# Artemarius/cuda-gaussian-splatting

Measured on AMD Instinct MI355X. Metric: fwd+bwd Mpixels/s @1080p, 1M Gaussians, SH3, higher is better.
Workload: dtype f32

## Files before the change

### cuda-gaussian-splatting_amd/csrc/cugs_gaussian_math.h

```cpp
#pragma once

#include "cugs_common.h"

struct V3 { float x, y, z; };
struct Sym2 { float a, b, c; };
struct Sym3 { float xx, xy, xz, yy, yz, zz; };
struct M3 { float m00, m01, m02, m10, m11, m12, m20, m21, m22; };
struct M23 { float r0x, r0y, r0z, r1x, r1y, r1z; };

struct GradMoments { float m1x, m1y, m2xx, m2xy, m2yy; };
struct Grad2D { float mx, my, a, b, c; };
__device__ __forceinline__ Grad2D grads_from_moments(const GradMoments& m, float a, float b, float c) {
    Grad2D g;
    g.mx = a * m.m1x + b * m.m1y;
    g.my = b * m.m1x + c * m.m1y;
    g.a = -0.5f * m.m2xx;
    g.b = -m.m2xy;
    g.c = -0.5f * m.m2yy;
    return g;
}

__device__ __forceinline__ M3 view_rotation(const CamArgs& c) {
    return M3{c.view[0], c.view[1], c.view[2], c.view[4], c.view[5], c.view[6],
              c.view[8], c.view[9], c.view[10]};
}

__device__ __forceinline__ V3 to_camera(const CamArgs& c, const M3& W, V3 p) {
    V3 t;
    t.x = W.m00 * p.x + W.m01 * p.y + W.m02 * p.z + c.view[3];
    t.y = W.m10 * p.x + W.m11 * p.y + W.m12 * p.z + c.view[7];
    t.z = W.m20 * p.x + W.m21 * p.y + W.m22 * p.z + c.view[11];
    return t;
}

struct QuatRot { M3 R; float inv_norm, w, x, y, z; };
__device__ __forceinline__ QuatRot rotation_of(float w, float x, float y, float z) {
    QuatRot o;
    o.inv_norm = cugs_rsqrtf(w * w + x * x + y * y + z * z + 1e-12f);
    w *= o.inv_norm; x *= o.inv_norm; y *= o.inv_norm; z *= o.inv_norm;
    o.w = w; o.x = x; o.y = y; o.z = z;
    o.R.m00 = 1.0f - 2.0f * (y * y + z * z);
    o.R.m01 = 2.0f * (x * y - w * z);
    o.R.m02 = 2.0f * (x * z + w * y);
    o.R.m10 = 2.0f * (x * y + w * z);
    o.R.m11 = 1.0f - 2.0f * (x * x + z * z);
    o.R.m12 = 2.0f * (y * z - w * x);
    o.R.m20 = 2.0f * (x * z - w * y);
    o.R.m21 = 2.0f * (y * z + w * x);
    o.R.m22 = 1.0f - 2.0f * (x * x + y * y);
    return o;
}

__device__ __forceinline__ M3 scale_columns(const M3& R, V3 s) {
    return M3{R.m00 * s.x, R.m01 * s.y, R.m02 * s.z, R.m10 * s.x, R.m11 * s.y, R.m12 * s.z,
              R.m20 * s.x, R.m21 * s.y, R.m22 * s.z};
}

__device__ __forceinline__ Sym3 gram(const M3& M) {
    Sym3 S;
    S.xx = M.m00 * M.m00 + M.m01 * M.m01 + M.m02 * M.m02;
    S.xy = M.m00 * M.m10 + M.m01 * M.m11 + M.m02 * M.m12;
    S.xz = M.m00 * M.m20 + M.m01 * M.m21 + M.m02 * M.m22;
    S.yy = M.m10 * M.m10 + M.m11 * M.m11 + M.m12 * M.m12;
    S.yz = M.m10 * M.m20 + M.m11 * M.m21 + M.m12 * M.m22;
    S.zz = M.m20 * M.m20 + M.m21 * M.m21 + M.m22 * M.m22;
    return S;
}

struct Jac { float j00, j02, j11, j12, tz_inv, tz_inv2; };
__device__ __forceinline__ Jac jacobian(V3 t, float fx, float fy) {
    Jac J;
    J.tz_inv = 1.0f / (t.z + 1e-6f);
    J.tz_inv2 = J.tz_inv * J.tz_inv;
    J.j00 = fx * J.tz_inv;
    J.j02 = -fx * t.x * J.tz_inv2;
    J.j11 = fy * J.tz_inv;
    J.j12 = -fy * t.y * J.tz_inv2;
    return J;
}

__device__ __forceinline__ M23 project_matrix_full(const Jac& J, const M3& W) {
    const float z = 0.0f;
    M23 T;
    T.r0x = J.j00 * W.m00 + z * W.m10 + J.j02 * W.m20;
    T.r0y = J.j00 * W.m01 + z * W.m11 + J.j02 * W.m21;
    T.r0z = J.j00 * W.m02 + z * W.m12 + J.j02 * W.m22;
    T.r1x = z * W.m00 + J.j11 * W.m10 + J.j12 * W.m20;
    T.r1y = z * W.m01 + J.j11 * W.m11 + J.j12 * W.m21;
    T.r1z = z * W.m02 + J.j11 * W.m12 + J.j12 * W.m22;
    return T;
}

__device__ __forceinline__ M23 project_matrix_sparse(const Jac& J, const M3& W) {
    M23 T;
    T.r0x = J.j00 * W.m00 + J.j02 * W.m20;
    T.r0y = J.j00 * W.m01 + J.j02 * W.m21;
    T.r0z = J.j00 * W.m02 + J.j02 * W.m22;
    T.r1x = J.j11 * W.m10 + J.j12 * W.m20;
    T.r1y = J.j11 * W.m11 + J.j12 * W.m21;
    T.r1z = J.j11 * W.m12 + J.j12 * W.m22;
    return T;
}

__device__ __forceinline__ M23 times_sym3(const M23& T, const Sym3& S) {
    M23 P;
    P.r0x = T.r0x * S.xx + T.r0y * S.xy + T.r0z * S.xz;
    P.r0y = T.r0x * S.xy + T.r0y * S.yy + T.r0z * S.yz;
    P.r0z = T.r0x * S.xz + T.r0y * S.yz + T.r0z * S.zz;
    P.r1x = T.r1x * S.xx + T.r1y * S.xy + T.r1z * S.xz;
    P.r1y = T.r1x * S.xy + T.r1y * S.yy + T.r1z * S.yz;
    P.r1z = T.r1x * S.xz + T.r1y * S.yz + T.r1z * S.zz;
    return P;
}

__device__ __forceinline__ Sym2 screen_covariance(const M23& T, const Sym3& S) {
    M23 P = times_sym3(T, S);
    Sym2 c;
    c.a = P.r0x * T.r0x + P.r0y * T.r0y + P.r0z * T.r0z;
    c.b = P.r0x * T.r1x + P.r0y * T.r1y + P.r0z * T.r1z;
    c.c = P.r1x * T.r1x + P.r1y * T.r1y + P.r1z * T.r1z;
    c.a += 0.3f;
    c.c += 0.3f;
    return c;
}

__device__ __forceinline__ int splat_radius(const Sym2& c) {
    float det = c.a * c.c - c.b * c.b;
    float trace = c.a + c.c;
    float disc = fmaxf(trace * trace - 4.0f * det, 0.0f);
    float lambda_max = 0.5f * (trace + sqrtf(disc));
    if (lambda_max <= 0.0f) return 0;
    return cugs_f2i(ceilf(3.0f * sqrtf(lambda_max)));
}

__device__ __forceinline__ float invert_sym2(const Sym2& c, Sym2& inv) {
    float det = c.a * c.c - c.b * c.b;
    if (det <= 0.0f) { inv = Sym2{0.0f, 0.0f, 0.0f}; return 0.0f; }
    float inv_det = 1.0f / det;
    inv.a = c.c * inv_det;
    inv.b = -c.b * inv_det;
    inv.c = c.a * inv_det;
    return det;
}

struct TileRect { int x0, y0, x1, y1; };
__device__ __forceinline__ TileRect tile_rect_of(float x, float y, int radius, int w, int h,
                                                 int ntx, int nty) {
    float rf = (float)radius;
    int min_x = max(0, cugs_f2i(x - rf));
    int min_y = max(0, cugs_f2i(y - rf));
    int max_x = min(w, cugs_f2i(x + rf + 1.0f));
    int max_y = min(h, cugs_f2i(y + rf + 1.0f));
    TileRect r;
    r.x0 = min_x / CUGS_TILE;
    r.y0 = min_y / CUGS_TILE;
    r.x1 = min(ntx, (max_x + CUGS_TILE - 1) / CUGS_TILE);
    r.y1 = min(nty, (max_y + CUGS_TILE - 1) / CUGS_TILE);
    return r;
}

constexpr int CUGS_DEPTH_BITS = 9;
constexpr uint32_t CUGS_DEPTH_KEY_BASE = 0x3E4CCCCCu;
constexpr uint32_t CUGS_DEPTH_KEY_SPAN = 1u << (3 * CUGS_DEPTH_BITS);
struct SortRecord { uint32_t key; int4 rect; };
__device__ __forceinline__ SortRecord sort_record_of(float depth, int tiles, int radius, TileRect tr, bool three_pass,
                                                     bool* out_of_range) {
    uint32_t key = __float_as_uint(depth);
    int x0 = 0, y0 = 0, w = 0, h = 0;
    if (tiles > 0) {
        if (radius > 0 && tr.x1 > tr.x0 && tr.y1 > tr.y0) {
            x0 = tr.x0; y0 = tr.y0; w = tr.x1 - tr.x0; h = tr.y1 - tr.y0;
        }
        if (w == 0) key = 0u;
    }
    *out_of_range = false;
    if (three_pass) {
        const uint32_t off = key - CUGS_DEPTH_KEY_BASE;
        const bool emits = tiles > 0 && w > 0;
        *out_of_range = emits && !(off >= 1u && off < CUGS_DEPTH_KEY_SPAN);
        key = emits ? min(off, CUGS_DEPTH_KEY_SPAN - 1u) : 0u;
    }
    return SortRecord{key, make_int4(x0, y0, w | (h << 16), tiles > 0 ? tiles : 0)};
}

constexpr int CUGS_PRECT_MAX_TILES = 127;
__host__ __device__ inline bool cugs_prect_packable(int ntx, int nty) { return ntx <= CUGS_PRECT_MAX_TILES && nty <= CUGS_PRECT_MAX_TILES; }
__device__ __forceinline__ uint32_t pack_rect(int4 r) {
    const int w = r.z & 0xFFFF, h = r.z >> 16;
    if (w == 0) return 0x80000000u | (uint32_t)r.w;
    return (uint32_t)r.x | ((uint32_t)r.y << 7) | ((uint32_t)w << 14) | ((uint32_t)h << 21);
}
__device__ __forceinline__ int4 unpack_rect(uint32_t v) {
    if (v & 0x80000000u) return make_int4(0, 0, 0, (int)(v & 0x7FFFFFFFu));
    const int x0 = (int)(v & 127u), y0 = (int)((v >> 7) & 127u), w = (int)((v >> 14) & 127u), h = (int)((v >> 21) & 127u);
    return make_int4(x0, y0, w | (h << 16), w * h);
}

__device__ __forceinline__ V3 view_direction(V3 p, const CamArgs& c) {
    float dx = p.x - c.cc[0], dy = p.y - c.cc[1], dz = p.z - c.cc[2];
    float nrm = fmaxf(sqrtf(dx * dx + dy * dy + dz * dz), 1e-8f);
    return V3{dx / nrm, dy / nrm, dz / nrm};
}

__device__ __forceinline__ void sh_basis(int degree, V3 d, float (&Y)[16]) {
    const float x = d.x, y = d.y, z = d.z;
    Y[0] = 0.28209479177387814f;
    if (degree >= 1) {
        Y[1] = -0.4886025119029199f * y;
        Y[2] = 0.4886025119029199f * z;
        Y[3] = -0.4886025119029199f * x;
    }
    if (degree >= 2) {
        const float xx = x * x, yy = y * y, zz = z * z;
        Y[4] = 1.0925484305920792f * (x * y);
        Y[5] = 1.0925484305920792f * (y * z);
        Y[6] = 0.31539156525252005f * (2 * zz - xx - yy);
        Y[7] = 1.0925484305920792f * (x * z);
        Y[8] = 0.5462742152960396f * (xx - yy);
    }
    if (degree >= 3) {
        const float xx = x * x, yy = y * y, zz = z * z;
        Y[9] = 0.5900435899266435f * y * (3 * xx - yy);
        Y[10] = 2.890611442640554f * x * y * z;
        Y[11] = 0.4570457994644658f * y * (4 * zz - xx - yy);
        Y[12] = 0.3731763325901154f * z * (2 * zz - 3 * xx - 3 * yy);
        Y[13] = 0.4570457994644658f * x * (4 * zz - xx - yy);
        Y[14] = 1.4453057213202769f * z * (xx - yy);
        Y[15] = 0.5900435899266435f * x * (xx - 3 * yy);
    }
}

__device__ __forceinline__ float raw_colour_backward(const float* c, const float (&Y)[16], int num_active) {
    float raw = 0.0f;
#pragma unroll
    for (int k = 0; k < 16; ++k)
        if (k < num_active) raw += c[k] * Y[k];
    return raw + 0.5f;
}

template <typename Ptr>
__device__ __forceinline__ float sh_colour(int degree, Ptr c, int stride, V3 d) {
    const float x = d.x, y = d.y, z = d.z;
    float color = 0.0f;
    color += 0.28209479177387814f * c[0];
    if (degree >= 1) {
        color += 0.4886025119029199f * (-c[1 * stride] * y + c[2 * stride] * z + -c[3 * stride] * x);
    }
    if (degree >= 2) {
        const float xx = x * x, yy = y * y, zz = z * z;
        const float xy = x * y, xz = x * z, yz = y * z;
        color += 1.0925484305920792f * c[4 * stride] * xy;
        color += 1.0925484305920792f * c[5 * stride] * yz;
        color += 0.31539156525252005f * c[6 * stride] * (2 * zz - xx - yy);
        color += 1.0925484305920792f * c[7 * stride] * xz;
        color += 0.5462742152960396f * c[8 * stride] * (xx - yy);
    }
    if (degree >= 3) {
        const float xx = x * x, yy = y * y, zz = z * z;
        color += 0.5900435899266435f * c[9 * stride] * y * (3 * xx - yy);
        color += 2.890611442640554f * c[10 * stride] * x * y * z;
        color += 0.4570457994644658f * c[11 * stride] * y * (4 * zz - xx - yy);
        color += 0.3731763325901154f * c[12 * stride] * z * (2 * zz - 3 * xx - 3 * yy);
        color += 0.4570457994644658f * c[13 * stride] * x * (4 * zz - xx - yy);
        color += 1.4453057213202769f * c[14 * stride] * z * (xx - yy);
        color += 0.5900435899266435f * c[15 * stride] * x * (xx - 3 * yy);
    }
    return color + 0.5f;
}

__device__ __forceinline__ void write_packed(float* packed, int64_t idx, float mx, float my,
                                             Sym2 inv, float r, float g, float b, float opacity) {
    float tau = (opacity >= (1.0f / 255.0f)) ? logf(255.0f * opacity) : -1.0f;
    float4* dst = reinterpret_cast<float4*>(packed + idx * CUGS_PACKED_STRIDE);
    dst[0] = make_float4(mx, my, inv.a, inv.b);
    dst[1] = make_float4(inv.c, opacity, tau, 0.0f);
    dst[2] = make_float4(r, 0.0f, g, b);
}
```

### cuda-gaussian-splatting_amd/csrc/sort_bin.h

```cpp
#pragma once

#include "sort_tile_order.h"

namespace {

constexpr int BIN_WAVES = 16, BIN_NT = BIN_WAVES * CUGS_WAVE;
inline uint32_t bin_window_groups(int ntx) { const uint32_t nbx = ((uint32_t)ntx + 7u) / 8u; return (nbx + 7u) / 8u; }
inline uint32_t bin_window_cols(int ntx) {
    const uint32_t nbx = ((uint32_t)ntx + 7u) / 8u, gxs = bin_window_groups(ntx);
    return ((nbx + gxs - 1u) / gxs) * 8u;
}
inline uint32_t bin_windows(int ntx, int nty) { return (((uint32_t)nty + 7u) / 8u) * bin_window_groups(ntx); }

constexpr int BIN_D_MAX = BIN_TILES_CAP + 2 * CUGS_PRECT_MAX_TILES + 2;
__global__ __launch_bounds__(BIN_NT) void k_bin_count(uint32_t n, uint32_t group, const uint32_t* __restrict__ order,
                                                      const int4* __restrict__ rect, const uint32_t* __restrict__ prect_in,
                                                      uint32_t* __restrict__ prect_out, uint32_t ntx, uint32_t nty,
                                                      uint32_t* __restrict__ table, uint32_t* __restrict__ zero_pairs,
                                                      uint32_t* __restrict__ win) {
    __shared__ int32_t s_d[BIN_D_MAX];
    if (blockIdx.x == 0 && threadIdx.x < BIN_WINDOWS_MAX) win[threadIdx.x] = 0u;
    __shared__ int32_t s_part[8][128];
    const uint32_t tid = threadIdx.x, wave = tid >> 6, lane = tid & 63u;
    const uint32_t w2 = ntx + 1u, cells = w2 * (nty + 1u);
    for (uint32_t e = tid; e < cells; e += BIN_NT) s_d[e] = 0;
    __syncthreads();
    const uint32_t base = blockIdx.x * group;
    const uint32_t end = min(n, base + group);
    for (uint32_t i = base + tid; i < end; i += BIN_NT) {
        uint32_t pr;
        if (prect_in) {
            pr = prect_in[i];
        } else {
            pr = pack_rect(rect[order[i]]);
            prect_out[i] = pr;
        }
        if (pr & 0x80000000u) {
            const uint32_t z = pr & 0x7FFFFFFFu;
            if (z) atomicAdd(zero_pairs, z);
            continue;
        }
        const uint32_t x0 = pr & 127u, y0 = (pr >> 7) & 127u, w = (pr >> 14) & 127u, h = (pr >> 21) & 127u;
        atomicAdd(&s_d[y0 * w2 + x0], 1);
        atomicAdd(&s_d[y0 * w2 + x0 + w], -1);
        atomicAdd(&s_d[(y0 + h) * w2 + x0], -1);
        atomicAdd(&s_d[(y0 + h) * w2 + x0 + w], 1);
    }
    __syncthreads();
    for (uint32_t row = wave; row < nty; row += BIN_WAVES) {
        int32_t carry = 0;
        for (uint32_t c0 = 0; c0 < ntx; c0 += CUGS_WAVE) {
            const uint32_t x = c0 + lane;
            const int32_t v = x < ntx ? s_d[row * w2 + x] : 0;
            const int32_t inc = (int32_t)wave_inclusive_scan((uint32_t)v) + carry;
            if (x < ntx) s_d[row * w2 + x] = inc;
            carry = __shfl(inc, 63);
        }
    }
    __syncthreads();
    {
        const uint32_t x = tid & 127u, seg = tid >> 7;
        const uint32_t rps = (nty + 7u) / 8u;
        const uint32_t ya = min(nty, seg * rps), yb = min(nty, ya + rps);
        int32_t sum = 0;
        if (x < ntx)
            for (uint32_t y = ya; y < yb; ++y) sum += s_d[y * w2 + x];
        s_part[seg][x] = sum;
        __syncthreads();
        int32_t run = 0;
        for (uint32_t s2 = 0; s2 < seg; ++s2) run += s_part[s2][x];
        if (x < ntx)
            for (uint32_t y = ya; y < yb; ++y) {
                run += s_d[y * w2 + x];
                s_d[y * w2 + x] = run;
            }
    }
    __syncthreads();
    uint32_t* out = table + (size_t)blockIdx.x * (ntx * nty);
    for (uint32_t row = wave; row < nty; row += BIN_WAVES)
        for (uint32_t x = lane; x < ntx; x += CUGS_WAVE) out[row * ntx + x] = (uint32_t)s_d[row * w2 + x];
}

__global__ __launch_bounds__(BIN_NT) void k_bin_scan(uint32_t rows, uint32_t tiles, uint32_t* __restrict__ table,
                                                     uint32_t* __restrict__ ttot, uint32_t* __restrict__ tpre,
                                                     uint32_t* __restrict__ csum, uint32_t* __restrict__ q12,
                                                     uint32_t* __restrict__ range_flag, uint32_t* __restrict__ snap,
                                                     uint32_t* __restrict__ win, uint32_t ntx, uint32_t win_cols,
                                                     uint32_t gxs) {
    __shared__ uint32_t s_seg[BIN_WAVES][CUGS_WAVE];
    __shared__ uint32_t s_win[BIN_WINDOWS_MAX];
    if (blockIdx.x == 0 && threadIdx.x == 0) {
        snap[0] = q12[0]; q12[1] = q12[0]; q12[0] = 0u;
        snap[1] = *range_flag; *range_flag = 0u;
    }
    const uint32_t tl = threadIdx.x & 63u, seg = threadIdx.x >> 6;
    const uint32_t t = blockIdx.x * CUGS_WAVE + tl;
    const uint32_t rps = (rows + BIN_WAVES - 1u) / BIN_WAVES;
    const uint32_t r0 = min(rows, seg * rps), r1 = min(rows, r0 + rps);
    uint32_t sum = 0u;
    if (t < tiles) {
#pragma unroll 8
        for (uint32_t r = r0; r < r1; ++r) sum += table[(size_t)r * tiles + t];
    }
    s_seg[seg][tl] = sum;
    __syncthreads();
    uint32_t pre = 0u, tot = 0u;
#pragma unroll
    for (uint32_t s2 = 0; s2 < (uint32_t)BIN_WAVES; ++s2) {
        const uint32_t v = s_seg[s2][tl];
        pre += s2 < seg ? v : 0u;
        tot += v;
    }
    if (t < tiles) {
        uint32_t run = pre;
#pragma unroll 8
        for (uint32_t r = r0; r < r1; ++r) {
            const uint32_t v = table[(size_t)r * tiles + t];
            table[(size_t)r * tiles + t] = run;
            run += v;
        }
    }
    if (seg == 0u) {
        const uint32_t v = t < tiles ? tot : 0u;
        const uint32_t inc = wave_inclusive_scan(v);
        if (t < tiles) { ttot[t] = v; tpre[t] = inc - v; }
        if (tl == 63u) csum[blockIdx.x] = inc;
        if (win) {
            s_win[tl] = 0u;
            __builtin_amdgcn_fence(__ATOMIC_ACQ_REL, "wavefront");
            __builtin_amdgcn_wave_barrier();
            if (v) {
                const uint32_t ty = t / ntx, tx = t - ty * ntx;
                atomicAdd(&s_win[(ty >> 3) * gxs + tx / win_cols], v);
            }
            __builtin_amdgcn_fence(__ATOMIC_ACQ_REL, "wavefront");
            __builtin_amdgcn_wave_barrier();
            const uint32_t mine = s_win[tl];
            if (mine) atomicAdd(&win[tl], mine);
        }
    }
}

constexpr int BIN_BLK = 8;
constexpr int BIN_WG_WAVES = 8;
constexpr int BIN_SLICE = 512;
constexpr int BIN_SLICE_STEPS = BIN_SLICE / CUGS_WAVE;
constexpr int BIN_RUN = 16;
constexpr int BIN_RUN_STRIDE = BIN_RUN + 3;
template <bool STAGE>
__global__ __launch_bounds__(BIN_WG_WAVES * CUGS_WAVE) void k_bin_scatter(
    uint32_t n, uint32_t group, uint32_t nbx, uint32_t nby, uint32_t gxs, uint32_t pairs_or_cap, bool predicted,
    const uint32_t* __restrict__ order, const uint32_t* __restrict__ prect, uint32_t ntx, uint32_t nty,
    const uint32_t* __restrict__ table, const uint32_t* __restrict__ ttot, const uint32_t* __restrict__ tpre,
    const uint32_t* __restrict__ csum, const uint32_t* __restrict__ snap, uint32_t* __restrict__ tbase,
    unsigned long long* __restrict__ total, unsigned long long* __restrict__ total_mapped, uint32_t* __restrict__ out,
    int32_t* __restrict__ tile_ranges, uint32_t* __restrict__ tile_order, const uint32_t* __restrict__ win) {
    __shared__ uint2 s_cand[BIN_WG_WAVES][BIN_SLICE];
    __shared__ uint32_t s_cnt[BIN_WG_WAVES];
    __shared__ uint32_t s_run[STAGE ? BIN_WG_WAVES * CUGS_WAVE * BIN_RUN_STRIDE + 4 : 1];
    const uint32_t nt = blockDim.x, nw = nt >> 6, tid = threadIdx.x, wid = tid >> 6, lane = tid & 63u;
    const uint32_t per_group = nby * gxs;
    uint32_t blk = blockIdx.x / per_group, rem = blockIdx.x - blk * per_group;
    const uint32_t win_mine = (win && lane < per_group) ? win[lane] : 0u;
    const uint32_t zero = snap[0];
    const bool bad = snap[1] != 0u;
    const uint32_t tiles = ntx * nty;

    const uint32_t nch = (tiles + CUGS_WAVE - 1u) / CUGS_WAVE;
    uint32_t cpre[3] = {0u, 0u, 0u};
    uint32_t pairs = zero;
#pragma unroll
    for (int i = 0; i < 3; ++i) {
        if ((uint32_t)i * CUGS_WAVE < nch) {
            const uint32_t c = lane + (uint32_t)i * CUGS_WAVE;
            const uint32_t v = c < nch ? csum[c] : 0u;
            uint32_t inc = v;
#pragma unroll
            for (int d = 1; d < 64; d <<= 1) {
                const uint32_t o = __shfl_up(inc, d);
                const uint32_t sum = inc + o;
                if ((int)lane >= d) inc = sum < o ? 0xFFFFFFFFu : sum;
            }
            const uint32_t with = inc + pairs;
            cpre[i] = (with < inc ? 0xFFFFFFFFu : with) - v;
            const uint32_t last = __shfl(inc, 63), tot = last + pairs;
            pairs = tot < last ? 0xFFFFFFFFu : tot;
        }
    }
    const bool fits = !bad && (!predicted || pairs <= pairs_or_cap);
    cpre[0] -= zero; cpre[1] -= zero; cpre[2] -= zero;
    if (__ballot((unsigned long long)win_mine * per_group > 2ull * pairs) != 0ull) {
        uint32_t rank = 0u;
        for (uint32_t w2 = 0; w2 < per_group; ++w2) {
            const uint32_t o = (uint32_t)__builtin_amdgcn_readlane((int)win_mine, (int)w2);
            rank += (o > win_mine || (o == win_mine && w2 < lane)) ? 1u : 0u;
        }
        const uint32_t groups = gridDim.x / per_group;
        const uint32_t slot = blockIdx.x / groups;
        blk = blockIdx.x - slot * groups;
        rem = (uint32_t)__builtin_ctzll(__ballot(lane < per_group && rank == slot));
    }
    const uint32_t by = rem / gxs, gx = rem - by * gxs;

    const uint32_t bx = gx * nw + wid;
    const bool active = bx < nbx;
    const uint32_t tx = bx * BIN_BLK + (lane & 7u), ty = by * BIN_BLK + (lane >> 3);
    const bool tile_ok = active && tx < ntx && ty < nty;
    const uint32_t t = tile_ok ? ty * ntx + tx : 0u;
    uint32_t start;
    {
        const uint32_t ch = t >> 6;
        const uint32_t p0 = __shfl(cpre[0], ch & 63u), p1 = __shfl(cpre[1], ch & 63u), p2 = __shfl(cpre[2], ch & 63u);
        start = zero + (ch < 64u ? p0 : ch < 128u ? p1 : p2) + (tile_ok ? tpre[t] : 0u);
    }
    uint32_t pos = tile_ok ? (start + table[(size_t)blk * tiles + t]) * 4u : 0u;
    if (blk == 0u) {
        if (tile_ok) {
            const uint32_t c = fits ? ttot[t] + (t == 0u ? zero : 0u) : 0u;
            tile_ranges[2 * t + 0] = c ? (int32_t)(t == 0u ? 0u : start) : 0;
            tile_ranges[2 * t + 1] = c ? (int32_t)(start + ttot[t]) : 0;
            tbase[t] = start;
        }
        if (rem == 0u && tid == 0u) {
            unsigned long long exact = zero;
            for (uint32_t c = 0; c < nch; ++c) exact += csum[c];
            tbase[tiles] = pairs;
            const unsigned long long host_total = bad ? ~0ull : exact;
            total[0] = bad ? 0ull : exact;
            total[1] = host_total;
            if (total_mapped) __hip_atomic_store(total_mapped, host_total, __ATOMIC_RELAXED, __HIP_MEMORY_SCOPE_SYSTEM);
        }
    }
    if (tile_order && blockIdx.x == 0u) {
        uint32_t* const s_lds = reinterpret_cast<uint32_t*>(&s_cand[0][0]);
        uint32_t* const s_chunk = s_lds + ORDER_LDS;
        if (wid == 0u) {
#pragma unroll
            for (int i = 0; i < 3; ++i)
                if (lane + (uint32_t)i * CUGS_WAVE < nch) s_chunk[lane + (uint32_t)i * CUGS_WAVE] = cpre[i];
        }
        write_tile_order(tiles, [&](uint32_t t2) { return fits ? ttot[t2] + (t2 == 0u ? zero : 0u) : 0u; },
                         [&](uint32_t t2) { return t2 == 0u ? 0u : zero + s_chunk[t2 >> 6] + tpre[t2]; },
                         reinterpret_cast<uint4*>(tile_order), s_lds);
    }
    if (!fits) return;
    if (blk == 0u)
        for (uint32_t k = rem * nt + tid; k < zero; k += per_group * nt) out[k] = 0u;
    const uint32_t win_y0 = by * BIN_BLK, win_y1 = win_y0 + BIN_BLK;
    const uint32_t win_x0 = gx * nw * BIN_BLK, win_x1 = win_x0 + nw * BIN_BLK;
    const uint32_t blk_x0 = bx * BIN_BLK, blk_x1 = blk_x0 + BIN_BLK;
    const unsigned long long lt_mask = (1ull << lane) - 1ull;
    char* const outb = reinterpret_cast<char*>(out);
    uint32_t* const run = s_run + (STAGE ? tid * BIN_RUN_STRIDE : 0u);
    uint32_t held = 0u;
    const uint32_t base = blk * group;
    const uint32_t end = min(n, base + group);
    const uint32_t stage = nw * BIN_SLICE;
    for (uint32_t c0 = base; c0 < end; c0 += stage) {
        __syncthreads();
        {
            const uint32_t s_begin = c0 + wid * BIN_SLICE;
            uint32_t pr[BIN_SLICE_STEPS], gq[BIN_SLICE_STEPS];
            bool ov[BIN_SLICE_STEPS];
#pragma unroll
            for (int u = 0; u < BIN_SLICE_STEPS; ++u) {
                const uint32_t i = s_begin + (uint32_t)u * CUGS_WAVE + lane;
                pr[u] = prect[min(i, end - 1u)];
                gq[u] = order[min(i, end - 1u)];
                if (i >= end) pr[u] = 0x80000000u;
            }
#pragma unroll
            for (int u = 0; u < BIN_SLICE_STEPS; ++u) {
                const uint32_t x0 = pr[u] & 127u, y0 = (pr[u] >> 7) & 127u, w = (pr[u] >> 14) & 127u, h = (pr[u] >> 21) & 127u;
                ov[u] = (int32_t)pr[u] >= 0 && y0 < win_y1 && y0 + h > win_y0 && x0 < win_x1 && x0 + w > win_x0;
            }
            uint32_t found = 0u;
#pragma unroll
            for (int u = 0; u < BIN_SLICE_STEPS; ++u) {
                const unsigned long long m = __ballot(ov[u]);
                if (ov[u]) s_cand[wid][found + (uint32_t)__popcll(m & lt_mask)] = make_uint2(pr[u], gq[u]);
                found += (uint32_t)__popcll(m);
            }
            if (lane == 0u) s_cnt[wid] = found;
        }
        __syncthreads();
        if (!active) continue;
        for (uint32_t w2 = 0; w2 < nw; ++w2) {
            const uint32_t c = s_cnt[w2];
            for (uint32_t k0 = 0; k0 < c; k0 += CUGS_WAVE) {
                uint2 rec = make_uint2(0x80000000u, 0u);
                if (k0 + lane < c) rec = s_cand[w2][k0 + lane];
                const uint32_t x0v = rec.x & 127u, wv = (rec.x >> 14) & 127u;
                unsigned long long m = __ballot((int32_t)rec.x >= 0 && x0v < blk_x1 && x0v + wv > blk_x0);
                while (m != 0ull) {
                    const int l = __builtin_ctzll(m);
                    m &= m - 1ull;
                    const uint32_t prl = (uint32_t)__builtin_amdgcn_readlane((int)rec.x, l);
                    const uint32_t g = (uint32_t)__builtin_amdgcn_readlane((int)rec.y, l);
                    const uint32_t x0 = prl & 127u, y0 = (prl >> 7) & 127u, w = (prl >> 14) & 127u, h = (prl >> 21) & 127u;
                    const bool in = ((tx - x0) < w) & ((ty - y0) < h);
                    if constexpr (STAGE) {
                        if (in) run[held++] = g;
                        if (__ballot(held == (uint32_t)BIN_RUN) != 0ull) {
                            const uint32_t whole = held & ~3u;
#pragma unroll
                            for (int q = 0; q < BIN_RUN; q += 4)
                                if ((uint32_t)q < whole)
                                    *reinterpret_cast<uint4*>(outb + pos + 4 * q) = make_uint4(run[q], run[q + 1], run[q + 2], run[q + 3]);
                            const uint32_t rest = held - whole;
                            const uint32_t r0 = run[whole], r1 = run[whole + 1u], r2 = run[whole + 2u];
                            if (rest > 0u) run[0] = r0;
                            if (rest > 1u) run[1] = r1;
                            if (rest > 2u) run[2] = r2;
                            pos += 4u * whole;
                            held = rest;
                        }
                    } else if (in) {
                        *reinterpret_cast<uint32_t*>(outb + pos) = g;
                        pos += 4u;
                    }
                }
            }
        }
    }
    if constexpr (STAGE) {
        for (uint32_t q = 0; __ballot(q < held) != 0ull; ++q)
            if (q < held) *reinterpret_cast<uint32_t*>(outb + pos + 4u * q) = run[q];
    }
}

__global__ __launch_bounds__(CUGS_BLOCK) void k_bin_keys(uint32_t pairs_or_cap, const unsigned long long* __restrict__ dev_count,
                                                         uint32_t tiles, const uint32_t* __restrict__ tbase,
                                                         const uint32_t* __restrict__ zero_snap,
                                                         const int32_t* __restrict__ pidx, const float* __restrict__ depths,
                                                         uint64_t* __restrict__ keys_sorted) {
    if (dev_count && *dev_count > (unsigned long long)pairs_or_cap) return;
    const uint32_t total = live_count(pairs_or_cap, dev_count);
    const uint32_t i = blockIdx.x * CUGS_BLOCK + threadIdx.x;
    if (i >= total) return;
    if (i < *zero_snap) { keys_sorted[i] = 0ull; return; }
    uint32_t lo = 0u, hi = tiles;
    while (hi - lo > 1u) {
        const uint32_t mid = (lo + hi) >> 1;
        if (tbase[mid] <= i) lo = mid; else hi = mid;
    }
    keys_sorted[i] = ((uint64_t)lo << 32) | (uint64_t)__float_as_uint(depths[pidx[i]]);
}

}
```

Measured before the change: 2611.

## Pack tile rects into SWAR byte words and hand-schedule the scatter hit loop

Candidate rectangles are re-encoded as byte-packed bound words, so the tile-in-rect and span-overlap tests become one subtract-and-mask instead of several field extractions and compares. The non-staged scatter inner loop is replaced with inline assembly (ff1, readlane, SWAR test, exec-masked store) to shorten the per-hit instruction sequence. The chunk prefix scan now runs once in wave 0 and goes through LDS, replacing per-wave scans and shuffles, at the cost of an extra barrier. Debug-only slot guards and a probe counter are added under CUGS_DEV.

```diff
diff --git a/cuda-gaussian-splatting_amd/csrc/cugs_bin_words.h b/cuda-gaussian-splatting_amd/csrc/cugs_bin_words.h
--- /dev/null
+++ b/cuda-gaussian-splatting_amd/csrc/cugs_bin_words.h
@@ -0,0 +1,29 @@
+#pragma once
+
+#include <stdint.h>
+
+#if defined(__HIPCC__)
+#define CUGS_BIN_HD __host__ __device__ __forceinline__
+#else
+#define CUGS_BIN_HD static inline
+#endif
+
+constexpr uint32_t CUGS_BIN_TOP_BITS = 0x80808080u, CUGS_BIN_INSIDE = 0x00008080u;
+constexpr uint32_t CUGS_BIN_NO_RECT = 0u, CUGS_BIN_NO_TILE = 0x8080807Fu;
+
+CUGS_BIN_HD uint32_t cugs_bin_tile_word(uint32_t tx, uint32_t ty) {
+    return (tx + 128u) * 0x00010001u | (ty + 128u) * 0x01000100u;
+}
+CUGS_BIN_HD uint32_t cugs_bin_rect_word(uint32_t packed) {
+    const uint32_t x0 = packed & 127u, y0 = (packed >> 7) & 127u, w = (packed >> 14) & 127u, h = (packed >> 21) & 127u;
+    return x0 | y0 << 8 | (x0 + w) << 16 | (y0 + h) << 24;
+}
+CUGS_BIN_HD bool cugs_bin_inside(uint32_t tile_word, uint32_t rect_word) {
+    return ((tile_word - rect_word) & CUGS_BIN_TOP_BITS) == CUGS_BIN_INSIDE;
+}
+CUGS_BIN_HD uint32_t cugs_bin_span_word(uint32_t xa, uint32_t xb) {
+    return (xb + 127u) | (xa + 128u) << 16 | 0xFF00FF00u;
+}
+CUGS_BIN_HD bool cugs_bin_overlaps_span(uint32_t span_word, uint32_t rect_word) {
+    return ((span_word - rect_word) & 0x00800080u) == 0x00000080u;
+}
diff --git a/cuda-gaussian-splatting_amd/csrc/cugs_gaussian_math.h b/cuda-gaussian-splatting_amd/csrc/cugs_gaussian_math.h
--- a/cuda-gaussian-splatting_amd/csrc/cugs_gaussian_math.h
+++ b/cuda-gaussian-splatting_amd/csrc/cugs_gaussian_math.h
@@ -1,6 +1,7 @@
 #pragma once
 
 #include "cugs_common.h"
+#include "cugs_bin_words.h"
 
 struct V3 { float x, y, z; };
 struct Sym2 { float a, b, c; };
diff --git a/cuda-gaussian-splatting_amd/csrc/sort_bin.h b/cuda-gaussian-splatting_amd/csrc/sort_bin.h
--- a/cuda-gaussian-splatting_amd/csrc/sort_bin.h
+++ b/cuda-gaussian-splatting_amd/csrc/sort_bin.h
@@ -145,8 +145,36 @@
 constexpr int BIN_WG_WAVES = 8;
 constexpr int BIN_SLICE = 512;
 constexpr int BIN_SLICE_STEPS = BIN_SLICE / CUGS_WAVE;
+constexpr uint32_t BIN_CHUNKS_MAX = 3u * CUGS_WAVE;
+static_assert(BIN_TILES_CAP <= (int)BIN_CHUNKS_MAX * CUGS_WAVE, "the scatter scans the chunk sums in three steps");
+static_assert(ORDER_LDS + BIN_CHUNKS_MAX + 1u <= 2u * BIN_SLICE, "tile order + chunk prefixes + total fit one wave's candidate list");
 constexpr int BIN_RUN = 16;
 constexpr int BIN_RUN_STRIDE = BIN_RUN + 3;
+__device__ __forceinline__ unsigned long long bin_clear_bit(unsigned long long m, int l) {
+    asm("s_bitset0_b64 %0, %1" : "+s"(m) : "s"(l));
+    return m;
+}
+__device__ __forceinline__ void bin_walk_hit(unsigned long long& m, uint32_t rect_word, uint32_t gaussian, uint32_t tile_word,
+                                             uint32_t& pos, char* outb) {
+    uint32_t l, c, g, t;
+    unsigned long long keep;
+    asm volatile(
+        "s_ff1_i32_b64 %[l], %[m]\n\t"
+        "v_readlane_b32 %[c], %[cw], %[l]\n\t"
+        "v_readlane_b32 %[g], %[cg], %[l]\n\t"
+        "s_bitset0_b64 %[m], %[l]\n\t"
+        "v_subrev_u32 %[t], %[c], %[tw]\n\t"
+        "v_and_b32 %[t], 0x80808080, %[t]\n\t"
+        "v_cmp_eq_u32 vcc, 0x8080, %[t]\n\t"
+        "s_and_saveexec_b64 %[keep], vcc\n\t"
+        "v_mov_b32 %[t], %[g]\n\t"
+        "v_add_u32 %[pos], 4, %[pos]\n\t"
+        "global_store_dword %[pos], %[t], %[out] offset:-4\n\t"
+        "s_mov_b64 exec, %[keep]"
+        : [m] "+s"(m), [pos] "+v"(pos), [l] "=&s"(l), [c] "=&s"(c), [g] "=&s"(g), [t] "=&v"(t), [keep] "=&s"(keep)
+        : [cw] "v"(rect_word), [cg] "v"(gaussian), [tw] "v"(tile_word), [out] "s"(outb)
+        : "vcc", "memory");
+}
 template <bool STAGE>
 __global__ __launch_bounds__(BIN_WG_WAVES * CUGS_WAVE) void k_bin_scatter(
     uint32_t n, uint32_t group, uint32_t nbx, uint32_t nby, uint32_t gxs, uint32_t pairs_or_cap, bool predicted,
@@ -167,28 +195,38 @@
     const uint32_t tiles = ntx * nty;
 
     const uint32_t nch = (tiles + CUGS_WAVE - 1u) / CUGS_WAVE;
-    uint32_t cpre[3] = {0u, 0u, 0u};
-    uint32_t pairs = zero;
-#pragma unroll
-    for (int i = 0; i < 3; ++i) {
-        if ((uint32_t)i * CUGS_WAVE < nch) {
-            const uint32_t c = lane + (uint32_t)i * CUGS_WAVE;
-            const uint32_t v = c < nch ? csum[c] : 0u;
-            uint32_t inc = v;
-#pragma unroll
-            for (int d = 1; d < 64; d <<= 1) {
-                const uint32_t o = __shfl_up(inc, d);
-                const uint32_t sum = inc + o;
-                if ((int)lane >= d) inc = sum < o ? 0xFFFFFFFFu : sum;
-            }
-            const uint32_t with = inc + pairs;
-            cpre[i] = (with < inc ? 0xFFFFFFFFu : with) - v;
-            const uint32_t last = __shfl(inc, 63), tot = last + pairs;
-            pairs = tot < last ? 0xFFFFFFFFu : tot;
-        }
-    }
+    uint32_t* const s_lds = reinterpret_cast<uint32_t*>(&s_cand[0][0]);
+    uint32_t* const s_chunk = s_lds + ORDER_LDS;
+    uint32_t* const s_pairs = s_chunk + BIN_CHUNKS_MAX;
+    if (wid == 0u) {
+        uint32_t cpre[3] = {0u, 0u, 0u};
+        uint32_t pairs = zero;
+#pragma unroll
+        for (int i = 0; i < 3; ++i) {
+            if ((uint32_t)i * CUGS_WAVE < nch) {
+                const uint32_t c = lane + (uint32_t)i * CUGS_WAVE;
+                const uint32_t v = c < nch ? csum[c] : 0u;
+                uint32_t inc = v;
+#pragma unroll
+                for (int d = 1; d < 64; d <<= 1) {
+                    const uint32_t o = __shfl_up(inc, d);
+                    const uint32_t sum = inc + o;
+                    if ((int)lane >= d) inc = sum < o ? 0xFFFFFFFFu : sum;
+                }
+                const uint32_t with = inc + pairs;
+                cpre[i] = (with < inc ? 0xFFFFFFFFu : with) - v;
+                const uint32_t last = __shfl(inc, 63), tot = last + pairs;
+                pairs = tot < last ? 0xFFFFFFFFu : tot;
+            }
+        }
+#pragma unroll
+        for (int i = 0; i < 3; ++i)
+            if (lane + (uint32_t)i * CUGS_WAVE < nch) s_chunk[lane + (uint32_t)i * CUGS_WAVE] = cpre[i] - zero;
+        if (lane == 0u) s_pairs[0] = pairs;
+    }
+    __syncthreads();
+    const uint32_t pairs = s_pairs[0];
     const bool fits = !bad && (!predicted || pairs <= pairs_or_cap);
-    cpre[0] -= zero; cpre[1] -= zero; cpre[2] -= zero;
     if (__ballot((unsigned long long)win_mine * per_group > 2ull * pairs) != 0ull) {
         uint32_t rank = 0u;
         for (uint32_t w2 = 0; w2 < per_group; ++w2) {
@@ -207,13 +245,18 @@
     const uint32_t tx = bx * BIN_BLK + (lane & 7u), ty = by * BIN_BLK + (lane >> 3);
     const bool tile_ok = active && tx < ntx && ty < nty;
     const uint32_t t = tile_ok ? ty * ntx + tx : 0u;
-    uint32_t start;
-    {
-        const uint32_t ch = t >> 6;
-        const uint32_t p0 = __shfl(cpre[0], ch & 63u), p1 = __shfl(cpre[1], ch & 63u), p2 = __shfl(cpre[2], ch & 63u);
-        start = zero + (ch < 64u ? p0 : ch < 128u ? p1 : p2) + (tile_ok ? tpre[t] : 0u);
-    }
+    const uint32_t start = zero + s_chunk[t >> 6] + (tile_ok ? tpre[t] : 0u);
     uint32_t pos = tile_ok ? (start + table[(size_t)blk * tiles + t]) * 4u : 0u;
+#ifdef CUGS_DEV
+    static_assert(offsetof(SortCtl, snap_q12) - offsetof(SortCtl, probe_word) == 2 * sizeof(uint32_t), "probe word = snap - 2");
+    uint32_t* const probe = const_cast<uint32_t*>(snap) - 2;
+    const uint32_t next_run = blk + 1u < gridDim.x / per_group ? (tile_ok ? table[(size_t)(blk + 1u) * tiles + t] : 0u)
+                                                               : (tile_ok ? ttot[t] : 0u);
+    const uint32_t slot_end = tile_ok ? (start + next_run) * 4u : 0u;
+#define BIN_SLOT_GUARD(cond) && (cond)
+#else
+#define BIN_SLOT_GUARD(cond)
+#endif
     if (blk == 0u) {
         if (tile_ok) {
             const uint32_t c = fits ? ttot[t] + (t == 0u ? zero : 0u) : 0u;
@@ -232,13 +275,6 @@
         }
     }
     if (tile_order && blockIdx.x == 0u) {
-        uint32_t* const s_lds = reinterpret_cast<uint32_t*>(&s_cand[0][0]);
-        uint32_t* const s_chunk = s_lds + ORDER_LDS;
-        if (wid == 0u) {
-#pragma unroll
-            for (int i = 0; i < 3; ++i)
-                if (lane + (uint32_t)i * CUGS_WAVE < nch) s_chunk[lane + (uint32_t)i * CUGS_WAVE] = cpre[i];
-        }
         write_tile_order(tiles, [&](uint32_t t2) { return fits ? ttot[t2] + (t2 == 0u ? zero : 0u) : 0u; },
                          [&](uint32_t t2) { return t2 == 0u ? 0u : zero + s_chunk[t2 >> 6] + tpre[t2]; },
                          reinterpret_cast<uint4*>(tile_order), s_lds);
@@ -248,7 +284,8 @@
         for (uint32_t k = rem * nt + tid; k < zero; k += per_group * nt) out[k] = 0u;
     const uint32_t win_y0 = by * BIN_BLK, win_y1 = win_y0 + BIN_BLK;
     const uint32_t win_x0 = gx * nw * BIN_BLK, win_x1 = win_x0 + nw * BIN_BLK;
-    const uint32_t blk_x0 = bx * BIN_BLK, blk_x1 = blk_x0 + BIN_BLK;
+    const uint32_t tile_word = tile_ok ? cugs_bin_tile_word(tx, ty) : CUGS_BIN_NO_TILE;
+    const uint32_t span_word = cugs_bin_span_word(bx * BIN_BLK, bx * BIN_BLK + BIN_BLK);
     const unsigned long long lt_mask = (1ull << lane) - 1ull;
     char* const outb = reinterpret_cast<char*>(out);
     uint32_t* const run = s_run + (STAGE ? tid * BIN_RUN_STRIDE : 0u);
@@ -278,7 +315,7 @@
 #pragma unroll
             for (int u = 0; u < BIN_SLICE_STEPS; ++u) {
                 const unsigned long long m = __ballot(ov[u]);
-                if (ov[u]) s_cand[wid][found + (uint32_t)__popcll(m & lt_mask)] = make_uint2(pr[u], gq[u]);
+                if (ov[u]) s_cand[wid][found + (uint32_t)__popcll(m & lt_mask)] = make_uint2(cugs_bin_rect_word(pr[u]), gq[u]);
                 found += (uint32_t)__popcll(m);
             }
             if (lane == 0u) s_cnt[wid] = found;
@@ -288,24 +325,27 @@
         for (uint32_t w2 = 0; w2 < nw; ++w2) {
             const uint32_t c = s_cnt[w2];
             for (uint32_t k0 = 0; k0 < c; k0 += CUGS_WAVE) {
-                uint2 rec = make_uint2(0x80000000u, 0u);
+                uint2 rec = make_uint2(CUGS_BIN_NO_RECT, 0u);
                 if (k0 + lane < c) rec = s_cand[w2][k0 + lane];
-                const uint32_t x0v = rec.x & 127u, wv = (rec.x >> 14) & 127u;
-                unsigned long long m = __ballot((int32_t)rec.x >= 0 && x0v < blk_x1 && x0v + wv > blk_x0);
+                unsigned long long m = __ballot(cugs_bin_overlaps_span(span_word, rec.x));
                 while (m != 0ull) {
+#ifndef CUGS_DEV
+                    if constexpr (!STAGE) {
+                        bin_walk_hit(m, rec.x, rec.y, tile_word, pos, outb);
+                        continue;
+                    }
+#endif
                     const int l = __builtin_ctzll(m);
-                    m &= m - 1ull;
-                    const uint32_t prl = (uint32_t)__builtin_amdgcn_readlane((int)rec.x, l);
+                    const uint32_t rw = (uint32_t)__builtin_amdgcn_readlane((int)rec.x, l);
                     const uint32_t g = (uint32_t)__builtin_amdgcn_readlane((int)rec.y, l);
-                    const uint32_t x0 = prl & 127u, y0 = (prl >> 7) & 127u, w = (prl >> 14) & 127u, h = (prl >> 21) & 127u;
-                    const bool in = ((tx - x0) < w) & ((ty - y0) < h);
+                    const bool in = cugs_bin_inside(tile_word, rw);
                     if constexpr (STAGE) {
                         if (in) run[held++] = g;
                         if (__ballot(held == (uint32_t)BIN_RUN) != 0ull) {
                             const uint32_t whole = held & ~3u;
 #pragma unroll
                             for (int q = 0; q < BIN_RUN; q += 4)
-                                if ((uint32_t)q < whole)
+                                if ((uint32_t)q < whole BIN_SLOT_GUARD(pos + 4u * (uint32_t)q + 16u <= slot_end))
                                     *reinterpret_cast<uint4*>(outb + pos + 4 * q) = make_uint4(run[q], run[q + 1], run[q + 2], run[q + 3]);
                             const uint32_t rest = held - whole;
                             const uint32_t r0 = run[whole], r1 = run[whole + 1u], r2 = run[whole + 2u];
@@ -315,18 +355,24 @@
                             pos += 4u * whole;
                             held = rest;
                         }
-                    } else if (in) {
-                        *reinterpret_cast<uint32_t*>(outb + pos) = g;
+                    } else if (in BIN_SLOT_GUARD(pos < slot_end)) {
                         pos += 4u;
+                        *reinterpret_cast<uint32_t*>(outb + (size_t)pos - 4u) = g;
                     }
+                    m = bin_clear_bit(m, l);
                 }
             }
         }
     }
     if constexpr (STAGE) {
         for (uint32_t q = 0; __ballot(q < held) != 0ull; ++q)
-            if (q < held) *reinterpret_cast<uint32_t*>(outb + pos + 4u * q) = run[q];
-    }
+            if (q < held BIN_SLOT_GUARD(pos + 4u * q < slot_end)) *reinterpret_cast<uint32_t*>(outb + pos + 4u * q) = run[q];
+    }
+#ifdef CUGS_DEV
+    const unsigned long long astray = __ballot(pos + (STAGE ? 4u * held : 0u) != slot_end);
+    if (astray != 0ull && lane == 0u) atomicAdd(probe, (uint32_t)__popcll(astray));
+#endif
+#undef BIN_SLOT_GUARD
 }
 
 __global__ __launch_bounds__(CUGS_BLOCK) void k_bin_keys(uint32_t pairs_or_cap, const unsigned long long* __restrict__ dev_count,
```

After: 2625, median of 6. No clear change (+0.6%).
